# kokizzu/dragonboat

Hardware: AMD Instinct MI355X
Metric: committed entries/sec (node) at 1M active 3-replica groups, 16B payload; %HBM BW (higher is better)
Workload: dtype u64

## Files before the change

dragonboat_amd/abi.py:

```python
import ctypes as C

DRB_MAX_REPLICAS = 8
DRB_RI_DEPTH = 4
DRB_NONE = 0xFFFFFFFF

DRB_OK = 0
DRB_EINVAL = -1
DRB_EDEVICE = -2
DRB_ENOMEM = -3
DRB_ENOSYS = -4
DRB_ERANGE = -5
DRB_EAGAIN = -6
DRB_EDIVERTED = -7

MSG = dict(
    LocalTick=0, Election=1, LeaderHeartbeat=2, ConfigChangeEvent=3, NoOP=4,
    Ping=5, Pong=6, Propose=7, SnapshotStatus=8, Unreachable=9,
    CheckQuorum=10, BatchedReadIndex=11, Replicate=12, ReplicateResp=13,
    RequestVote=14, RequestVoteResp=15, InstallSnapshot=16, Heartbeat=17,
    HeartbeatResp=18, ReadIndex=19, ReadIndexResp=20, Quiesce=21,
    SnapshotReceived=22, LeaderTransfer=23, TimeoutNow=24, RateLimit=25,
    RequestPreVote=26, RequestPreVoteResp=27, LogQuery=28)
MSG_NAME = {v: k for k, v in MSG.items()}

# ... 77 lines not shown
                ("hint_high", C.c_uint64), ("type", C.c_uint32),
                ("reject", C.c_uint32), ("n_entries", C.c_uint64),
                ("entries_off", C.c_uint64)]


class ReadyToRead(C.Structure):
    _fields_ = [("shard_id", C.c_uint64), ("replica_id", C.c_uint64),
                ("index", C.c_uint64), ("ctx_low", C.c_uint64),
                ("ctx_high", C.c_uint64)]


class Config(C.Structure):
    _fields_ = [("num_groups", C.c_uint64), ("first_shard_id", C.c_uint64),
                ("num_replicas", C.c_uint32), ("window", C.c_uint32),
                ("cmd_cap", C.c_uint32), ("max_props", C.c_uint32),
                ("prop_slots", C.c_uint32), ("ri_slots", C.c_uint32),
                ("mailbox", C.c_uint32), ("kv_slots", C.c_uint32),
                ("kv_val_cap", C.c_uint32), ("election_rtt", C.c_uint32),
                ("heartbeat_rtt", C.c_uint32), ("check_quorum", C.c_uint32),
                ("device", C.c_int32), ("save_cap", C.c_uint32),
                ("total_groups", C.c_uint64), ("place_world", C.c_uint32),
                ("place_rank", C.c_uint32), ("entry_mbox", C.c_uint32),
                ("kv_pool_blocks", C.c_uint32), ("flagged_cap", C.c_uint32),
                ("quiesce", C.c_uint32), ("durable_log", C.c_uint32),
                ("save_batched", C.c_uint32), ("save_tan", C.c_uint32),
                ("elections", C.c_uint32), ("tan_max_log", C.c_uint64),
                ("tan_multiplexed", C.c_uint32), ("pre_vote", C.c_uint32),
                ("max_reads_per_ctx", C.c_uint32),
                ("kv_overflow_buckets", C.c_uint64),
                ("forward_proposals", C.c_uint32),
                ("nonvoting_slots", C.c_uint32),
                ("witness_slots", C.c_uint32),
                ("host_copies", C.c_uint32), ("no_lean", C.c_uint32),
                ("entry_compression", C.c_uint32),
                ("session_slots", C.c_uint32),
                ("session_history", C.c_uint32)]


class ReadResult(C.Structure):
    _fields_ = [("shard_id", C.c_uint64), ("index", C.c_uint64),
                ("ctx_low", C.c_uint64), ("ctx_high", C.c_uint64),
                ("key", C.c_uint64), ("replica_id", C.c_uint32),
                ("read", C.c_uint32), ("found", C.c_uint32),
                ("vlen", C.c_uint32), ("value", C.c_uint32),
                ("pad", C.c_uint32)]


class ApplyResult(C.Structure):
    _fields_ = [("group", C.c_uint64), ("index", C.c_uint64),
                ("key", C.c_uint64), ("client_id", C.c_uint64),
                ("series_id", C.c_uint64), ("value", C.c_uint64),
                ("slot", C.c_uint32), ("ignored", C.c_uint32)]


APPLY_IGNORED, APPLY_REJECTED = 1, 2

SERIES_REGISTER, SERIES_UNREGISTER = 2 ** 64 - 2, 2 ** 64 - 1


class SessionRec(C.Structure):
    _fields_ = [("client_id", C.c_uint64), ("responded_up_to", C.c_uint64),
                ("n_history", C.c_uint32), ("first_history", C.c_uint32)]


class SessionResp(C.Structure):
    _fields_ = [("series_id", C.c_uint64), ("value", C.c_uint64)]
# ... 224 lines not shown
```

dragonboat_amd/csrc/drb_engine.hip:

```cpp
#include <hip/hip_runtime.h>
#include <stdio.h>
#include <stdlib.h>
#include <string.h>

#include <algorithm>
#include <memory>
#include <mutex>
#include <unordered_map>
#include <vector>

#include <hipcub/hipcub.hpp>

#include "../../include/drb_engine.h"
#include "drb_layout.hpp"
#include "drb_msg.hpp"
#include "drb_place.hpp"
#include "drb_rows.hpp"
#include "drb_step.hpp"
#include "drb_launch.hpp"
#include "drb_hsa.hpp"
#include "drb_res.hpp"

using namespace drb;

#define HIPCHK(x)                                                        \
  do {                                                                   \
    hipError_t e_ = (x);                                                 \
    if (e_ != hipSuccess) {                                              \
      fprintf(stderr, "drb_engine: %s failed: %s (%s:%d)\n", #x,          \
              hipGetErrorString(e_), __FILE__, __LINE__);                \
      return DRB_EDEVICE;                                                \
    }                                                                    \
  } while (0)

struct drb_engine {
  drb_config cfg;
  View v;
  View *dview;
  Stream stream;
  Stream stream2;
  Event ev_fork, ev_join;
  Stream stream_h2d;
  HsaXfer xfer;
  int failed = 0;
  DevBuf sess_client;
  bool no_lean = false;
  std::vector<drb_engine *> bound;
  std::vector<PeerPlanes> peers_host;
  Event ev_staged;
  Event ev_stage_free;
  Event ev_uploaded;
  Event ev_xsend, ev_xrecv;
  uint64_t exchanged_round = 0;
  std::vector<Event> ev_prop;
  uint64_t round = 0;
  uint64_t ticks = 0;
  uint64_t committed_round = 0;
  uint64_t bytes = 0;
  std::vector<DevBuf> allocs;
  uint64_t ctr_rows = 0;
  uint32_t *xcount = nullptr;
  uint32_t role_slots[2] = {0, 0};
  uint32_t *role_dev = nullptr;
  unsigned long long *ctr_total = nullptr;
  DevBuf scratch;
  DevBuf stage_buf;
  struct WireState *wire = nullptr;
  struct IngestState *ingest = nullptr;
  struct WorkerState *worker = nullptr;
  std::mutex ingest_mu;
  bool crc_tab_ready = false;
  uint64_t tan_blocks = 0;
  uint64_t tan_wblocks = 0;
  uint32_t *tan_list = nullptr;
  uint32_t *tan_n = nullptr;
  uint32_t tan_per_list = 0;
  unsigned long long *tan_total = nullptr;
  uint64_t reads_round = ~0ull;
  uint32_t reads_n = 0, reads_ks = 0;
  DevBuf xout;
  unsigned long long *xpull_bytes = nullptr;
  uint64_t xcopy_bytes = 0;
  bool xrows_used = false;
  std::vector<bool> recovered;
};

static void wire_free(drb_engine *e);
// ... 104 lines not shown
  if (cfg->cmd_cap == 0 || cfg->cmd_cap % 16 || cfg->cmd_cap > 1040)
    return DRB_ENOSYS;
  if (cfg->mailbox < 4 || cfg->mailbox > MB_MAX) return DRB_EINVAL;
  if (!is_pow2(cfg->kv_slots) || cfg->kv_val_cap == 0 ||
      cfg->kv_val_cap > 1024)
    return DRB_EINVAL;
  if (cfg->max_props == 0 || cfg->prop_slots == 0 || cfg->ri_slots == 0)
    return DRB_EINVAL;
  if (cfg->save_cap % 16) return DRB_EINVAL;
  if (cfg->save_batched && (cfg->save_cap == 0 || cfg->window < 64))
    return DRB_EINVAL;
  if (cfg->save_tan && (cfg->save_cap == 0 || cfg->save_batched))
    return DRB_EINVAL;
  if (cfg->pre_vote && !cfg->elections) return DRB_EINVAL;
  if (cfg->tan_multiplexed && (!cfg->save_tan || cfg->place_world > 1))
    return DRB_EINVAL;
  if (cfg->save_tan && (uint64_t)cfg->num_replicas * cfg->num_groups > 0xffffffffull)
    return DRB_ERANGE;
  if (cfg->place_world > 1 &&
      (cfg->place_rank >= cfg->place_world || cfg->entry_mbox == 0 ||
       cfg->entry_mbox > cfg->window || cfg->entry_mbox > 255))
    return DRB_EINVAL;
  if (cfg->election_rtt == 0 || cfg->heartbeat_rtt == 0) return DRB_EINVAL;
  if ((cfg->nonvoting_slots & cfg->witness_slots) ||
      ((cfg->nonvoting_slots | cfg->witness_slots) >> cfg->num_replicas) ||
      __builtin_popcount(cfg->nonvoting_slots | cfg->witness_slots) >=
          (int)cfg->num_replicas)
    return DRB_EINVAL;
  if (cfg->forward_proposals &&
      (cfg->max_props > MAX_FWD_PROPS || cfg->place_world > 1))
    return DRB_EINVAL;
  if ((uint64_t)cfg->window * (128 + cfg->cmd_cap) > MAX_ENTRY_SIZE)
    return DRB_EINVAL;
  if (cfg->host_copies > 1 || cfg->entry_compression > 1) return DRB_EINVAL;
  if (cfg->session_slots > SESS_MAX_SLOTS ||
      (cfg->session_slots ? cfg->session_history == 0 ||
                                cfg->session_history > SESS_MAX_HISTORY
                          : cfg->session_history != 0))
    return DRB_EINVAL;
  if (cfg->total_groups >
      cfg->num_groups * std::max<uint64_t>(cfg->place_world, 1))
    return DRB_EINVAL;
  if (cfg->kv_overflow_buckets >= 0xffffffffull) return DRB_ERANGE;
  if (cfg->save_tan && cfg->tan_multiplexed &&
      (uint64_t)tanm_records(cfg->num_groups) * cfg->save_cap > 0xffffffffull)
    return DRB_ERANGE;
  return DRB_OK;
}

namespace {
struct EngineDestroy {
  void operator()(drb_engine *e) const { (void)drb_engine_destroy(e); }
};
}

extern "C" int drb_engine_create(const drb_config *cfg, drb_engine **out) {
  if (!cfg || !out) return DRB_EINVAL;
  *out = nullptr;
  if (int rc = validate_config(cfg)) return rc;
  std::unique_ptr<drb_engine, EngineDestroy> owner(new drb_engine());
  drb_engine *e = owner.get();
  e->cfg = *cfg;
  if (cfg->host_copies) e->xfer.state = -1;
  e->no_lean = cfg->no_lean != 0;
  if (hipSetDevice(cfg->device) != hipSuccess ||
      e->stream.create() != hipSuccess || e->stream2.create() != hipSuccess ||
      e->stream_h2d.create() != hipSuccess)
    return DRB_EDEVICE;
  e->ev_prop.resize(cfg->prop_slots);
  for (Event *ev : {&e->ev_fork, &e->ev_join, &e->ev_staged, &e->ev_stage_free,
                    &e->ev_uploaded, &e->ev_xsend, &e->ev_xrecv})
    if (ev->create() != hipSuccess) return DRB_EDEVICE;
  for (Event &ev : e->ev_prop)
    if (ev.create() != hipSuccess) return DRB_EDEVICE;
  View &v = e->v;
  memset(&v, 0, sizeof(v));
  const uint64_t G = cfg->num_groups, R = cfg->num_replicas;
  v.G = G;
  v.R = (uint32_t)R;
  v.W = cfg->window;
  v.C16 = cfg->cmd_cap / 16;
  v.MB = cfg->mailbox;
  v.KS = cfg->kv_slots;
  v.kv_val_cap = cfg->kv_val_cap;
  v.kv_ool = cfg->kv_val_cap > 124;
  v.KVW = v.kv_ool ? 2
                   : 1 + (cfg->kv_val_cap > 4 ? (cfg->kv_val_cap - 4 + 15) / 16
                                              : 0);
  v.VB = v.kv_ool ? (cfg->kv_val_cap + 15) / 16 : 0;
  v.kv_pool_blocks =
      v.kv_ool ? (cfg->kv_pool_blocks
                      ? cfg->kv_pool_blocks
                      : std::min<uint64_t>(G * R * v.KS +
                                               4 * cfg->kv_overflow_buckets,
                                           0xffffffffull))
               : 0;
  v.max_props = cfg->max_props;
  v.election_rtt = cfg->election_rtt;
  v.heartbeat_rtt = cfg->heartbeat_rtt;
// ... 674 lines not shown
  if (!e || slot >= e->v.R) return DRB_EINVAL;
  k_host_slot<<<(unsigned)((e->v.G + 255) / 256), 256, 0, e->stream>>>(
      e->v, slot, hosted ? 1u : 0u);
  HIPCHK(hipGetLastError());
  return refresh_roles(e);
}

DRB_DEV void stage_row(const View &v, uint32_t slot, uint32_t j, uint64_t g,
                       const drb_entry &en, const uint8_t *cmd,
                       bool readable) {
  uint4 meta[PROP_META];
  const bool held = prop_pack(v, en, cmd, readable, meta);
  for (uint32_t c = 0; c < PROP_META; ++c)
    v.props[prop_ix(v, slot, j, c, g)] = meta[c];
  for (uint32_t c = 0; held && c < v.C16; ++c)
    v.props[prop_ix(v, slot, j, PROP_META + c, g)] =
        cmd_chunk(cmd, en.cmd_len, c);
}

__global__ void k_stage_props(View v, uint32_t slot, const uint32_t *counts,
                              const drb_entry *ents, const uint8_t *pool,
                              uint64_t pool_len) {
  const uint64_t g = (uint64_t)blockIdx.x * blockDim.x + threadIdx.x;
  if (g >= v.G) return;
  const uint32_t n = counts[g];
  v.prop_count[(uint64_t)slot * v.G + g] = n;
  for (uint32_t j = 0; j < n; ++j) {
    const drb_entry en = ents[g * v.max_props + j];
    stage_row(v, slot, j, g, en, pool + en.cmd_off,
              en.cmd_off + en.cmd_len <= pool_len);
  }
}

extern "C" int drb_stage_proposals(drb_engine *e, uint32_t slot,
                                   const uint32_t *counts,
                                   const drb_entry *ents,
                                   const uint8_t *pool, size_t pool_len) {
  if (!e || slot >= e->cfg.prop_slots) return DRB_ERANGE;
  if (!counts || !ents || (pool_len && !pool)) return DRB_EINVAL;
  const View &v = e->v;
  const uint64_t G = v.G;
  for (uint64_t g = 0; g < G; ++g)
    if (counts[g] > v.max_props) return DRB_ERANGE;
  const size_t ent_b = (size_t)G * v.max_props * sizeof(drb_entry);
  const size_t cnt_off = ent_b, pool_off = (cnt_off + G * 4 + 255) & ~(size_t)255;
  const size_t need = pool_off + std::max<uint64_t>(pool_len, 16);
  if (need > e->stage_buf.cap) {
    HIPCHK(hipStreamSynchronize(e->stream));
    HIPCHK(hipStreamSynchronize(e->stream_h2d));
    if (e->stage_buf.reserve(need)) return DRB_EDEVICE;
  }
  uint8_t *d = e->stage_buf.as<uint8_t>();
  HIPCHK(hipStreamWaitEvent(e->stream_h2d, e->ev_stage_free, 0));
  HIPCHK(hipMemcpyAsync(d, ents, ent_b, hipMemcpyHostToDevice,
                        e->stream_h2d));
  HIPCHK(hipMemcpyAsync(d + cnt_off, counts, G * 4, hipMemcpyHostToDevice,
                        e->stream_h2d));
  if (pool_len)
    HIPCHK(hipMemcpyAsync(d + pool_off, pool, pool_len, hipMemcpyHostToDevice,
                          e->stream_h2d));
  HIPCHK(hipEventRecord(e->ev_staged, e->stream_h2d));
  HIPCHK(hipStreamWaitEvent(e->stream, e->ev_staged, 0));
  k_stage_props<<<(unsigned)((G + 255) / 256), 256, 0, e->stream>>>(
      v, slot, (const uint32_t *)(d + cnt_off), (const drb_entry *)d,
      d + pool_off, (uint64_t)pool_len);
  HIPCHK(hipGetLastError());
  HIPCHK(hipEventRecord(e->ev_stage_free, e->stream));
  HIPCHK(hipEventRecord(e->ev_prop[slot], e->stream));
  HIPCHK(hipEventSynchronize(e->ev_staged));
  return DRB_OK;
}

// ... 29 lines not shown
  }
}

constexpr size_t kSdmaMinBytes = 8u << 20;

static void stage_layout(uint64_t G, uint64_t n, size_t pool_len,
                         uint64_t off[4], size_t *bytes) {
  auto al = [](size_t x) { return (x + 255) & ~(size_t)255; };
  const uint64_t n1 = n ? n : 1;
  off[0] = al(G);
  off[2] = off[0] + al(8 * n1);
  off[3] = off[2] + al(2 * n1);
  off[1] = al(off[3] + pool_len);
  *bytes = off[1] + 8 * n1;
}

extern "C" int drb_stage_packed_layout(const drb_engine *e, uint64_t n_entries,
                                       size_t pool_len, uint64_t *offsets,
                                       size_t *bytes) {
  if (!e || !offsets || !bytes) return DRB_EINVAL;
  stage_layout(e->v.G, n_entries, pool_len, offsets, bytes);
  return DRB_OK;
}

static int stage_packed(drb_engine *e, uint32_t slot, uint32_t type,
                        const uint8_t *counts, uint64_t n_entries,
                        const uint64_t *keys, const uint64_t *client_ids,
                        const uint16_t *cmd_lens, const uint8_t *pool,
                        size_t pool_len, bool async) {
  if (!e || slot >= e->cfg.prop_slots) return DRB_ERANGE;
  if (!counts || (n_entries && (!keys || !cmd_lens)) || (pool_len && !pool))
    return DRB_EINVAL;
  if (n_entries && !client_ids && !e->sess_client.p) return DRB_EINVAL;
  const View &v = e->v;
  const uint64_t G = v.G, n = n_entries;
  uint64_t tsum = 0;
  uint32_t cmax = 0;
  for (uint64_t g = 0; g < G; ++g) {
    cmax = std::max<uint32_t>(cmax, counts[g]);
    tsum += counts[g];
  }
  if (cmax > v.max_props) return DRB_ERANGE;
  if (tsum != n) return DRB_EINVAL;
  auto al = [](size_t x) { return (x + 255) & ~(size_t)255; };
  const uint64_t n1 = n ? n : 1;
  size_t tb1 = 0, tb2 = 0;
  HIPCHK(hipcub::DeviceScan::ExclusiveSum(
      nullptr, tb1, WidenU8((const uint8_t *)nullptr, WidenU32()),
      (uint32_t *)nullptr, (int)G, e->stream));
  HIPCHK(hipcub::DeviceScan::ExclusiveSum(
      nullptr, tb2, WidenU16((const uint16_t *)nullptr, WidenU32()),
      (uint32_t *)nullptr, (int)n1, e->stream));
  uint64_t lo[4];
  size_t up = 0;
  stage_layout(G, n, pool_len, lo, &up);
  const size_t o_cnt = 0, o_key = lo[0], o_cid = lo[1], o_len = lo[2],
               o_pool = lo[3];
  if (!client_ids) up = o_pool + pool_len;
  const size_t o_e0 = al(std::max<size_t>(up, o_pool + 16)),
               o_off = o_e0 + al(4 * G), o_tmp = o_off + al(4 * n1),
               need = o_tmp + al(std::max(tb1, tb2));
  if (need > e->stage_buf.cap) {
    HIPCHK(hipStreamSynchronize(e->stream));
    HIPCHK(hipStreamSynchronize(e->stream_h2d));
    if (e->stage_buf.reserve(need)) return DRB_EDEVICE;
  }
// ... 182 lines not shown
      const bool on =
          mix64(seed ^ ACTIVE_SALT ^ (g * 0x9E3779B97F4A7C15ull) ^
                (salt << 24)) % 1000000u < active_ppm;
      v.prop_count[(uint64_t)ps * v.G + lane] = on ? k : 0u;
      if (on) list[atomicAdd(&nlist, 1u)] = (uint32_t)(lane - base);
    }
    __syncthreads();
    const uint32_t n = nlist;
    if (n >= 256 || it + 1 == GEN_ITERS) {
      if (threadIdx.x < n && threadIdx.x < 256)
        gen_kv_lane(v, ps, k, key_space, val_len, seed, salt,
                    base + list[threadIdx.x]);
      __syncthreads();
      if (n > 256 && threadIdx.x < n - 256)
        list[threadIdx.x] = list[256 + threadIdx.x];
      if (threadIdx.x == 0) nlist = n > 256 ? n - 256 : 0u;
      __syncthreads();
    }
  }
  const uint32_t n = nlist;
  if (threadIdx.x < n)
    gen_kv_lane(v, ps, k, key_space, val_len, seed, salt,
                base + list[threadIdx.x]);
}

extern "C" int drb_gen_kv_proposals_active(drb_engine *e, uint32_t slot,
                                           uint32_t k, uint32_t key_space,
                                           uint32_t val_len, uint64_t seed,
                                           uint64_t salt, uint32_t active_ppm) {
  if (!e || slot >= e->cfg.prop_slots || k > e->cfg.max_props || !key_space ||
      val_len > 16383 ||
      12 + (val_len < 128 ? 1 : 2) + val_len > e->cfg.cmd_cap)
    return DRB_EINVAL;
  const uint64_t per = active_ppm >= 1000000u ? 256 : GEN_ITERS * 256;
  k_gen_kv<<<(unsigned)((e->v.G + per - 1) / per), 256, 0, e->stream>>>(
      e->v, slot, k, key_space, val_len, seed, salt, active_ppm);
  HIPCHK(hipGetLastError());
  HIPCHK(hipEventRecord(e->ev_prop[slot], e->stream));
  return DRB_OK;
}

extern "C" int drb_gen_kv_proposals(drb_engine *e, uint32_t slot, uint32_t k,
                                    uint32_t key_space, uint32_t val_len,
                                    uint64_t seed, uint64_t salt) {
  return drb_gen_kv_proposals_active(e, slot, k, key_space, val_len, seed,
                                     salt, 1000000u);
}

extern "C" int drb_stage_read_index(drb_engine *e, uint32_t slot,
                                    const uint64_t *ctx_low,
                                    const uint64_t *ctx_high) {
  if (!e || slot >= e->cfg.ri_slots) return DRB_ERANGE;
  const uint64_t G = e->v.G;
  std::vector<uint4> host(G);
  for (uint64_t g = 0; g < G; ++g) host[g] = pack2(ctx_low[g], ctx_high[g]);
  HIPCHK(hipMemcpyAsync(e->v.ri_in + (uint64_t)slot * G, host.data(),
                        G * sizeof(uint4), hipMemcpyHostToDevice, e->stream));
  HIPCHK(hipStreamSynchronize(e->stream));
  return DRB_OK;
}

__global__ void k_gen_ri(View v, uint32_t rs, uint64_t seed, uint64_t salt,
                         uint64_t high) {
  const uint64_t lane = (uint64_t)blockIdx.x * blockDim.x + threadIdx.x;
  if (lane >= v.G) return;
  const uint64_t g = gid(v, v.stage_slot, lane);
  uint64_t low = mix64(seed ^ 0x5EAD1DE85EAD1DE8ull ^
                       (g * 0x9E3779B97F4A7C15ull) ^ (salt << 40)) |
                 1;
  v.ri_in[(uint64_t)rs * v.G + lane] = mk4(low, high);
}
// ... 463 lines not shown
      for (int k = 0; k < NUM_STEP_KINDS; ++k)
        fn[R - 1][k] = fn[R - 1][step_kind_at(R, k)];
  }
};
static constexpr StepLaunchTable kStepLaunch;

static int launch_step(drb_engine *e, const RoundParams &p0,
                       hipStream_t st = nullptr, uint32_t blk0 = 0,
                       uint32_t nblk = 0) {
  const unsigned gx_all = (unsigned)((e->v.G + 255) / 256);
  const unsigned gx = nblk ? nblk : gx_all;
  if (!st) st = e->stream;
  if (e->v.R < 1 || e->v.R > 8) return DRB_EINVAL;
  if (p0.listed) {
    switch (e->v.R) {
#define DRB_X(R, K) \
  case R: k_active_scan<R><<<gx, 256, 0, e->stream>>>(e->v, p0); break;
      DRB_FOR_ALL_R(DRB_X, )
#undef DRB_X
    }
    k_active_prefix<<<4 * e->v.R, 1024, 0, e->stream>>>(e->v, gx);
    k_active_scatter<<<dim3(gx, e->v.R), 256, 0, e->stream>>>(e->v);
  }
  RoundParams pl = p0, pf = p0;
  pl.blk0 = pf.blk0 = blk0;
  pl.gx_all = pf.gx_all = nblk ? gx_all : 0u;
  uint32_t nl = 0, nf = 0;
  pl.slots = slot_list(e->role_slots[0], &nl);
  pf.slots = slot_list(e->role_slots[1], &nf);
  pl.nrows = nl;
  pf.nrows = nf;
  const StepPlan plan =
      plan_step(e->v, p0.encode_saves, p0.listed, nl, nf, gx,
                !nblk && st == e->stream, e->no_lean);
  const StepLaunchFn *launch = kStepLaunch.fn[e->v.R - 1];
  if (plan.split) {
    (void)hipEventRecord(e->ev_fork, st);
    (void)hipStreamWaitEvent(e->stream2, e->ev_fork, 0);
  }
  if (plan.lean) {
    if (plan.split) {
      (void)hipEventRecord(e->ev_join, e->stream2);
      (void)hipStreamWaitEvent(st, e->ev_join, 0);
    }
    if (nl) launch[SK_LEAD_LEAN](e->v, pl, gx * nl, st);
    if (nf) launch[SK_FOLLOW_LEAN](e->v, pf, gx * nf, st);
    pl.lean = pf.lean = LEAN_ALL;
    if (nl) launch[plan.lead](e->v, pl, gx * nl, st);
    if (nf) launch[plan.follow](e->v, pf, gx * nf, st);
  } else {
    if (nl) launch[plan.lead](e->v, pl, gx * nl, st);
    if (nf)
      launch[plan.follow](e->v, pf, gx * nf, plan.split ? e->stream2 : st);
    if (plan.split) {
      (void)hipEventRecord(e->ev_join, e->stream2);
      (void)hipStreamWaitEvent(st, e->ev_join, 0);
    }
    if (plan.slow) {
      RoundParams ps = p0;
      ps.slots = 0;
      ps.nrows = 1;
      launch[SK_SLOW](e->v, ps, (e->v.slow_cap + 255) / 256, e->stream);
    }
  }
  HIPCHK(hipGetLastError());
  return DRB_OK;
}
// ... 33 lines not shown
  __syncthreads();
  const uint64_t g = (uint64_t)blockIdx.x * blockDim.x + threadIdx.x;
  const uint32_t s = blockIdx.y;
  if (g < v.G) {
    const uint32_t fl = v.u32[u32_ix(v, W_FLAGS, s, g)];
    if ((fl & DRB_F_HOSTED) && !(fl & (DRB_F_FALLBACK | DRB_F_ERROR)))
      atomicAdd(&part[v.u32[u32_ix(v, W_ROLE, s, g)] & 7u], 1ull);
  }
  __syncthreads();
  if (threadIdx.x < 8 && part[threadIdx.x])
    atomicAdd(&out[s * 8 + threadIdx.x], part[threadIdx.x]);
}

extern "C" int drb_role_census(drb_engine *e, uint64_t *counts) {
  if (!e || !counts) return DRB_EINVAL;
  void *d;
  const size_t bytes = (size_t)e->v.R * 8 * sizeof(uint64_t);
  if (scratch(e, bytes, &d)) return DRB_EDEVICE;
  HIPCHK(hipMemsetAsync(d, 0, bytes, e->stream));
  dim3 grid((unsigned)((e->v.G + 255) / 256), e->v.R);
  k_role_census<<<grid, 256, 0, e->stream>>>(e->v,
                                             (unsigned long long *)d);
  HIPCHK(hipGetLastError());
  HIPCHK(hipMemcpyAsync(counts, d, bytes, hipMemcpyDeviceToHost, e->stream));
  HIPCHK(hipStreamSynchronize(e->stream));
  return DRB_OK;
}

extern "C" int drb_role_slots(const drb_engine *e, uint32_t *leader_slots,
                              uint32_t *follower_slots) {
  if (!e) return DRB_EINVAL;
  if (leader_slots) *leader_slots = e->role_slots[0];
  if (follower_slots) *follower_slots = e->role_slots[1];
  return DRB_OK;
}

static int round_params(drb_engine *e, const drb_round_in *in, uint64_t ahead,
                        uint64_t ticks_before, RoundParams *out) {
  if (in->prop_slot != DRB_NONE && in->prop_slot >= e->cfg.prop_slots)
    return DRB_ERANGE;
  if (in->ri_slot != DRB_NONE && in->ri_slot >= e->cfg.ri_slots)
    return DRB_ERANGE;
  RoundParams p;
  memset(&p, 0, sizeof(p));
  p.slots = 0;
  p.nrows = 1;
  p.round = e->round + 1 + ahead;
  p.tick = in->tick ? 1 : 0;
  p.tick_no = ticks_before + p.tick;
  p.prop_slot = in->prop_slot;
  p.ri_slot = in->ri_slot;
  p.n_reads = in->reads_per_ctx;
  p.key_space = in->read_key_space;
  if (p.n_reads && !p.key_space) return DRB_EINVAL;
  if (p.n_reads && e->v.max_reads && p.n_reads > e->v.max_reads)
    return DRB_ERANGE;
  p.encode_saves = in->encode_saves ? 1 : 0;
  if (p.encode_saves && !e->v.save_cap16) return DRB_EINVAL;
  p.ri_replica = in->ri_replica;
  p.listed = in->listed ? 1 : 0;
  if (p.listed && e->v.remote_mask) return DRB_EINVAL;
  p.prop_replica = in->prop_replica;
  if (p.prop_replica > e->v.R || (p.prop_replica && !e->v.fwd_props))
    return DRB_EINVAL;
  if (p.ri_replica > e->v.R || (p.ri_replica && e->v.place_world > 1))
    return DRB_EINVAL;
// ... 6 lines not shown

static void round_done(drb_engine *e, const RoundParams &p) {
  e->round++;
  e->ticks += p.tick;
  if (p.n_reads) {
    e->reads_round = e->round;
    e->reads_n = p.n_reads;
    e->reads_ks = p.key_space;
  }
}

extern "C" int drb_step_round_async(drb_engine *e, const drb_round_in *in) {
  if (!e || !in) return DRB_EINVAL;
  std::lock_guard<std::mutex> ingest_lock(e->ingest_mu);
  if (e->failed) return e->failed;
  if (e->cfg.durable_log && e->committed_round < e->round) return DRB_EINVAL;
  RoundParams p;
  if (int rc = round_params(e, in, 0, e->ticks, &p)) return rc;
  if (e->v.elections)
    HIPCHK(hipMemsetAsync(e->v.slow_n, 0, 8, e->stream));
  if (e->v.remote_mask && e->xrows_used)
    HIPCHK(hipMemsetAsync(e->v.xrows, 0,
                          2ull * e->v.R * e->v.R * ((e->v.G + 255) / 256) * 4,
                          e->stream));
  if (e->v.xslow && e->xrows_used)
    HIPCHK(hipMemsetAsync(e->v.xslow, 0,
                          4ull * e->v.R * e->v.R * ((e->v.G + 255) / 256) * 4,
                          e->stream));
  if (int rc = launch_step(e, p)) return rc;
  if (p.encode_saves && e->v.save_tan) {
    int rc = launch_tan(e, (uint32_t)p.round);
    if (rc) return rc;
  }
  if (p.prop_slot != DRB_NONE)
    HIPCHK(hipEventRecord(e->ev_prop[p.prop_slot], e->stream));
  round_done(e, p);
  return DRB_OK;
}

extern "C" int drb_step_rounds(drb_engine *e, const drb_round_in *in,
                               uint32_t k, uint64_t chunk_groups) {
  if (!e || !in || !k) return DRB_EINVAL;
  std::lock_guard<std::mutex> ingest_lock(e->ingest_mu);
  if (e->failed) return e->failed;
  if (e->v.elections || e->v.remote_mask || e->v.save_tan ||
      e->cfg.durable_log)
    return DRB_EINVAL;
  const uint64_t gx = (e->v.G + 255) / 256;
  if (!chunk_groups || chunk_groups % 256) return DRB_EINVAL;
  const uint64_t cb = chunk_groups / 256;
  std::vector<RoundParams> ps(k);
  uint64_t ticks = e->ticks;
  for (uint32_t t = 0; t < k; ++t) {
    if (in[t].listed) return DRB_EINVAL;
    if (int rc = round_params(e, &in[t], t, ticks, &ps[t])) return rc;
    ticks += ps[t].tick;
  }
  HIPCHK(hipEventRecord(e->ev_fork, e->stream));
  HIPCHK(hipStreamWaitEvent(e->stream2, e->ev_fork, 0));
  int rc = DRB_OK;
  if (cb >= gx) {
    for (uint32_t t = 0; t < k && !rc; ++t) rc = launch_step(e, ps[t]);
  } else {
    for (uint64_t c0 = 0, c = 0; c0 < gx && !rc; c0 += cb, ++c) {
      const uint32_t nb = (uint32_t)std::min<uint64_t>(cb, gx - c0);
      hipStream_t st = (c & 1) ? e->stream2 : e->stream;
      for (uint32_t t = 0; t < k && !rc; ++t)
        rc = launch_step(e, ps[t], st, (uint32_t)c0, nb);
    }
  }
  const hipError_t j1 = hipEventRecord(e->ev_join, e->stream2);
  const hipError_t j2 = hipStreamWaitEvent(e->stream, e->ev_join, 0);
  if (rc || j1 != hipSuccess || j2 != hipSuccess) {
    e->failed = rc ? rc : DRB_EDEVICE;
    return e->failed;
  }
  for (uint32_t t = 0; t < k; ++t) {
    if (ps[t].prop_slot != DRB_NONE)
      HIPCHK(hipEventRecord(e->ev_prop[ps[t].prop_slot], e->stream));
    round_done(e, ps[t]);
  }
  return DRB_OK;
}

__global__ void k_sum_counters(const unsigned long long *rows, uint64_t n,
                               unsigned long long *total) {
  __shared__ unsigned long long part[256];
  for (int c = 0; c < NUM_COUNTERS; ++c) {
    unsigned long long s = 0;
    for (uint64_t r = threadIdx.x; r < n; r += blockDim.x)
      s += rows[r * NUM_COUNTERS + c];
    part[threadIdx.x] = s;
    __syncthreads();
    for (int o = 128; o > 0; o >>= 1) {
      if (threadIdx.x < (unsigned)o) part[threadIdx.x] += part[threadIdx.x + o];
      __syncthreads();
    }
    if (threadIdx.x == 0) total[c] = part[0];
    __syncthreads();
  }
}

extern "C" int drb_debug_phase(drb_engine *e, uint64_t *out, int reset) {
  if (!e || !out) return DRB_EINVAL;
  memset(out, 0, 16 * sizeof(uint64_t));
  if (!e->v.phase) return DRB_OK;
  HIPCHK(hipMemcpyAsync(out, e->v.phase, 16 * sizeof(uint64_t),
                        hipMemcpyDeviceToHost, e->stream));
  if (reset)
    HIPCHK(hipMemsetAsync(e->v.phase, 0, 16 * sizeof(uint64_t), e->stream));
  HIPCHK(hipStreamSynchronize(e->stream));
  return DRB_OK;
// ... 2229 lines not shown
```

dragonboat_amd/csrc/drb_kinds.hpp:

```cpp
#pragma once
#include "drb_layout.hpp"

namespace drb {

#define DRB_FOR_ALL_R(X, K) \
  X(1, K) X(2, K) X(3, K) X(4, K) X(5, K) X(6, K) X(7, K) X(8, K)
#define DRB_FOR_R3_R5(X, K) X(3, K) X(5, K)

#define DRB_STEP_KINDS(X)                                                  \
  X(LEAD, 0, STEP, 1, 0, 0, 0, 0, ALL_R, LEAD)                             \
  X(LEAD_EXT, 1, STEP, 1, 1, 0, 0, 0, ALL_R, LEAD_EXT)                     \
  X(FOLLOW, 2, STEP, 0, 0, 0, 0, 0, ALL_R, FOLLOW)                         \
  X(FOLLOW_EXT, 3, STEP, 0, 1, 0, 0, 0, ALL_R, FOLLOW_EXT)                 \
  X(SLOW, 4, STEP, 1, 1, 1, 1, 0, ALL_R, SLOW)                             \
  X(LEAD_FWD, 5, STEP, 1, 1, 0, 1, 0, ALL_R, LEAD_FWD)                     \
  X(FOLLOW_FWD, 6, STEP, 0, 1, 0, 1, 0, ALL_R, FOLLOW_FWD)                 \
  X(LEAD_LEAN, 7, LEAN, 1, 0, 0, 0, 0, ALL_R, LEAD_LEAN)                   \
  X(FOLLOW_LEAN, 8, LEAN, 0, 0, 0, 0, 0, ALL_R, FOLLOW_LEAN)               \
  X(LEAD_LOCAL, 9, STEP, 1, 0, 0, 0, 1, R3_R5, LEAD)                       \
  X(FOLLOW_LOCAL, 10, STEP, 0, 0, 0, 0, 1, R3_R5, FOLLOW)                  \
  X(LEAD_EXT_LOCAL, 11, STEP, 1, 1, 0, 0, 1, R3_R5, LEAD_EXT)              \
  X(FOLLOW_EXT_LOCAL, 12, STEP, 0, 1, 0, 0, 1, R3_R5, FOLLOW_EXT)

enum StepKind : int {
#define DRB_X(name, num, ...) SK_##name = num,
  DRB_STEP_KINDS(DRB_X)
#undef DRB_X
  NUM_STEP_KINDS
};

enum StepKernel { SKN_STEP, SKN_LEAN };

struct StepKindInfo {
  StepKernel kernel;
  bool lead, ext, slow, fwd, local;
  uint32_t built_for;
  int stand_in;
};

constexpr StepKindInfo kStepKinds[NUM_STEP_KINDS] = {
#define DRB_X_BIT(R, K) | 1u << R
#define DRB_X(name, num, kernel, L, E, S, F, LOC, set, alt)              \
  {SKN_##kernel, L != 0, E != 0, S != 0, F != 0, LOC != 0,               \
   0u DRB_FOR_##set(DRB_X_BIT, num), SK_##alt},
    DRB_STEP_KINDS(DRB_X)
#undef DRB_X
#undef DRB_X_BIT
};

constexpr int step_kind_at(int R, int kind) {
  return (kStepKinds[kind].built_for >> R) & 1u ? kind
                                                : kStepKinds[kind].stand_in;
}

constexpr uint64_t kSplitMaxBlocks = 2048;

struct StepPlan {
  int lead, follow;
  bool split;
  bool lean;
  bool slow;
};

inline StepPlan plan_step(const View &v, bool encode_saves, bool listed,
                          uint32_t nl, uint32_t nf, unsigned gx,
                          bool whole_round_on_engine_stream, bool no_lean) {
  const bool ext = v.C16 > 4 || v.kv_ool || encode_saves || v.quiesce ||
                   v.kv_ovf_cap || v.snappy || v.sessions;
  const bool fwd = v.fwd_props || v.nv_mask || v.wt_mask;
  const bool local = !v.remote_mask;
  StepPlan p;
  p.lead = fwd ? SK_LEAD_FWD
           : ext ? (local ? SK_LEAD_EXT_LOCAL : SK_LEAD_EXT)
                 : (local ? SK_LEAD_LOCAL : SK_LEAD);
  p.follow = fwd ? SK_FOLLOW_FWD
             : ext ? (local ? SK_FOLLOW_EXT_LOCAL : SK_FOLLOW_EXT)
                   : (local ? SK_FOLLOW_LOCAL : SK_FOLLOW);
  p.split = nl && nf && whole_round_on_engine_stream && !v.elections &&
            (uint64_t)gx * (nl + nf) <= kSplitMaxBlocks;
  p.lean = listed && ext && !fwd && whole_round_on_engine_stream &&
           !v.elections && local && !v.save_tan && !v.save_batched &&
           !no_lean;
  p.slow = v.elections != 0;
  return p;
}

}
```

dragonboat_amd/csrc/drb_res.hpp:

```cpp
#pragma once

#include <stddef.h>

#include <utility>

namespace drb {

template <class A>
struct Buf {
  void *p = nullptr;
  size_t cap = 0;

  Buf() = default;
  Buf(Buf &&o) noexcept : p(o.p), cap(o.cap) { o.p = nullptr, o.cap = 0; }
  Buf &operator=(Buf &&o) noexcept {
    if (this != &o) {
      reset();
      std::swap(p, o.p);
      std::swap(cap, o.cap);
    }
    return *this;
  }
  ~Buf() { reset(); }

// ... 54 lines not shown
static inline int hip_alloc_rc(hipError_t r, const char *what, size_t bytes) {
  if (r != hipSuccess)
    fprintf(stderr, "drb_engine: %s of %zu bytes failed: %s\n", what, bytes,
            hipGetErrorString(r));
  return r != hipSuccess;
}
struct HipDevice {
  static int alloc(void **p, size_t n) {
    return hip_alloc_rc(hipMalloc(p, n), "hipMalloc", n);
  }
  static void free(void *p) { (void)hipFree(p); }
};
template <unsigned Flags>
struct HipPinned {
  static int alloc(void **p, size_t n) {
    return hip_alloc_rc(hipHostMalloc(p, n, Flags), "hipHostMalloc", n);
  }
  static void free(void *p) { (void)hipHostFree(p); }
};
using DevBuf = Buf<HipDevice>;
template <unsigned Flags>
using PinnedBuf = Buf<HipPinned<Flags>>;

struct StreamDestroy {
  static bool null(hipStream_t s) { return !s; }
  static void destroy(hipStream_t s) { (void)hipStreamDestroy(s); }
};
struct Stream : Handle<hipStream_t, StreamDestroy> {
  hipError_t create() {
    const hipError_t r = hipStreamCreateWithFlags(out(), hipStreamNonBlocking);
    if (r != hipSuccess) h = nullptr;
    return r;
  }
};
struct EventDestroy {
  static bool null(hipEvent_t e) { return !e; }
  static void destroy(hipEvent_t e) { (void)hipEventDestroy(e); }
};
struct Event : Handle<hipEvent_t, EventDestroy> {
  hipError_t create(unsigned flags = hipEventDisableTiming) {
    const hipError_t r = hipEventCreateWithFlags(out(), flags);
    if (r != hipSuccess) h = nullptr;
    return r;
  }
};
struct SignalDestroy {
  static bool null(hsa_signal_t s) { return !s.handle; }
  static void destroy(hsa_signal_t s) { (void)hsa_signal_destroy(s); }
};
struct Signal : Handle<hsa_signal_t, SignalDestroy> {
  hsa_status_t create() {
    const hsa_status_t r = hsa_signal_create(0, 0, nullptr, out());
    if (r != HSA_STATUS_SUCCESS) h = hsa_signal_t{0};
    return r;
  }
};

}
#endif
```

dragonboat_amd/engine.py:

```python
import ctypes as C
import os

from . import abi
from .abi import (ApplyResult, Config, Entry, Flagged, Message, ReadyToRead, Region, ReplicaState,
                  RoundIn, RoundOut, WireCfg, WireCpu, WireIn, WireOut,
                  entry_to_tuple,
                  message_to_tuple)

HERE = os.path.dirname(os.path.abspath(__file__))
LIB_PATH = os.environ.get("DRB_ENGINE_LIB") or \
    os.path.join(HERE, "_lib", "libdrb_engine.so")

_lib = None

P = C.c_void_p
U64 = C.c_uint64
U32 = C.c_uint32
PU64 = C.POINTER(C.c_uint64)
PU32 = C.POINTER(C.c_uint32)
PU8 = C.POINTER(C.c_uint8)
SZ = C.c_size_t

SIGNATURES = {
    "drb_engine_create": (C.c_int, [C.POINTER(Config), C.POINTER(P)]),
    "drb_engine_destroy": (C.c_int, [P]),
    "drb_engine_device_bytes": (U64, [P]),
    "drb_engine_stream": (P, [P]),
    "drb_engine_sync": (C.c_int, [P]),
    "drb_engine_round": (U64, [P]),
    "drb_import_replicas": (C.c_int, [P, U64, U64,
                                      C.POINTER(ReplicaState)]),
    "drb_export_replicas": (C.c_int, [P, U64, U64,
                                      C.POINTER(ReplicaState)]),
    "drb_import_log": (C.c_int, [P, U64, U32, C.POINTER(Entry), SZ, PU8]),
    "drb_export_log": (C.c_int, [P, U64, U32, U64, U64, C.POINTER(Entry),
                                 PU8, SZ]),
    "drb_init_steady": (C.c_int, [P, U64, U32, U64]),
    "drb_host_slot": (C.c_int, [P, U32, C.c_int]),
    "drb_role_census": (C.c_int, [P, PU64]),
    "drb_export_save_records": (C.c_int, [P, U64, U32,
                                          C.POINTER(abi.SaveRecord), SZ,
                                          C.POINTER(SZ)]),
    "drb_role_slots": (C.c_int, [P, PU32, PU32]),
    "drb_stage_proposals": (C.c_int, [P, U32, PU32, C.POINTER(Entry), PU8,
                                      SZ]),
    "drb_stage_proposals_packed": (C.c_int, [P, U32, U32, PU8, U64, PU64,
                                             PU64, C.POINTER(C.c_uint16),
                                             PU8, SZ]),
    "drb_stage_proposals_packed_async": (C.c_int, [P, U32, U32, PU8, U64, PU64,
                                             PU64, C.POINTER(C.c_uint16),
                                             PU8, SZ]),
    "drb_stage_wait_upload": (C.c_int, [P]),
    "drb_set_session_clients": (C.c_int, [P, PU64]),
    "drb_stage_packed_layout": (C.c_int, [P, U64, SZ, PU64, C.POINTER(SZ)]),
    "drb_gen_kv_proposals": (C.c_int, [P, U32, U32, U32, U32, U64, U64]),
    "drb_gen_kv_proposals_active": (C.c_int, [P, U32, U32, U32, U32, U64,
                                              U64, U32]),
    "drb_stage_read_index": (C.c_int, [P, U32, PU64, PU64]),
    "drb_gen_read_index": (C.c_int, [P, U32, U64, U64]),
    "drb_request_leader_transfer": (C.c_int, [P, U32, PU32, PU64]),
    "drb_ingest": (C.c_int, [P, C.POINTER(Message), SZ, C.POINTER(Entry),
                             PU8, PU64, PU64]),
    "drb_ingest_ex": (C.c_int, [P, C.POINTER(Message), SZ, C.POINTER(Entry),
                                PU8, PU8, PU64, PU64, PU64]),
    "drb_export_inbox": (C.c_int, [P, U64, U32, C.c_int, C.POINTER(Message),
                                   SZ, C.POINTER(Entry), SZ, PU8, SZ,
                                   C.POINTER(SZ)]),
    "drb_ingest_wire_cpu": (C.c_int, [P, C.POINTER(WireCpu), SZ,
                                      C.POINTER(SZ)]),
    "drb_step_round": (C.c_int, [P, C.POINTER(RoundIn),
                                 C.POINTER(RoundOut)]),
    "drb_step_round_async": (C.c_int, [P, C.POINTER(RoundIn)]),
    "drb_step_rounds": (C.c_int, [P, C.POINTER(RoundIn), U32, U64]),
    "drb_read_counters": (C.c_int, [P, C.POINTER(RoundOut), C.c_int]),
    "drb_debug_phase": (C.c_int, [P, C.POINTER(U64), C.c_int]),
    "drb_take_flagged": (C.c_int, [P, C.POINTER(Flagged), SZ, C.POINTER(SZ),
# ... 121 lines not shown
    n = SZ(0)
    _ck(lib().drb_payload_decode(type, _u8(cmd), len(cmd), out, cap,
                                 C.byref(n)), "drb_payload_decode")
    return bytes(out[:n.value])


def tan_scan(data, cap=None):
    data = bytes(data)
    n, oc, vend = SZ(0), C.c_int(0), U64(0)
    buf = _u8(data)
    want = 64 if cap is None else cap
    while True:
        out = (abi.TanScanRec * max(1, want))()
        _ck(lib().drb_tan_scan(buf, len(data), out, want, C.byref(n),
                               C.byref(oc), C.byref(vend)), "drb_tan_scan")
        if cap is not None or n.value <= want:
            break
        want = n.value
    recs = [{f: getattr(out[i], f) for f, _ in abi.TanScanRec._fields_}
            for i in range(min(n.value, want))]
    return oc.value, vend.value, recs


DEFAULTS = dict(num_groups=1, first_shard_id=1, num_replicas=3, window=32,
                cmd_cap=32, max_props=4, prop_slots=2, ri_slots=2,
                mailbox=16, kv_slots=512, kv_val_cap=4, election_rtt=10,
                heartbeat_rtt=1, check_quorum=1, device=0, save_cap=0,
                total_groups=0, place_world=1, place_rank=0, entry_mbox=0,
                kv_pool_blocks=0, flagged_cap=0, quiesce=0, durable_log=0,
                save_batched=0, save_tan=0, tan_max_log=0, elections=0,
                tan_multiplexed=0, pre_vote=0, max_reads_per_ctx=0,
                kv_overflow_buckets=0, forward_proposals=0,
                nonvoting_slots=0, witness_slots=0, host_copies=0,
                no_lean=0, entry_compression=0, session_slots=0,
                session_history=0)


class Engine:

    def __init__(self, **kw):
        cfg = dict(DEFAULTS)
        cfg.update(kw)
        self.cfg = cfg
        c = Config(cfg["num_groups"], cfg["first_shard_id"],
                   cfg["num_replicas"], cfg["window"], cfg["cmd_cap"],
                   cfg["max_props"], cfg["prop_slots"], cfg["ri_slots"],
                   cfg["mailbox"], cfg["kv_slots"], cfg["kv_val_cap"],
                   cfg["election_rtt"], cfg["heartbeat_rtt"],
                   cfg["check_quorum"], cfg["device"], cfg["save_cap"],
                   cfg["total_groups"], cfg["place_world"], cfg["place_rank"],
                   cfg["entry_mbox"], cfg["kv_pool_blocks"],
                   cfg["flagged_cap"], cfg["quiesce"],
                   cfg["durable_log"], cfg["save_batched"],
                   cfg["save_tan"], cfg["elections"], cfg["tan_max_log"],
                   cfg["tan_multiplexed"], cfg["pre_vote"],
                   cfg["max_reads_per_ctx"], cfg["kv_overflow_buckets"],
                   cfg["forward_proposals"], cfg["nonvoting_slots"],
                   cfg["witness_slots"], cfg["host_copies"],
                   cfg["no_lean"], cfg["entry_compression"],
                   cfg["session_slots"], cfg["session_history"])
        h = P()
        _ck(lib().drb_engine_create(C.byref(c), C.byref(h)),
            "drb_engine_create")
        self.h = h
        self.G = cfg["num_groups"]
        self.R = cfg["num_replicas"]

    def close(self):
        if getattr(self, "h", None):
            lib().drb_engine_destroy(self.h)
            self.h = None

    def __del__(self):
        self.close()

    @property
    def device_bytes(self):
        return lib().drb_engine_device_bytes(self.h)

    @property
    def round(self):
        return lib().drb_engine_round(self.h)

    @property
    def stream(self):
        return lib().drb_engine_stream(self.h)

    def sync(self):
        _ck(lib().drb_engine_sync(self.h), "drb_engine_sync")

    def import_replicas(self, first_group, states):
        n = len(states) // self.R
        arr = (ReplicaState * len(states))(*states)
        _ck(lib().drb_import_replicas(self.h, first_group, n, arr),
            "drb_import_replicas")

    def export_replicas(self, first_group, n_groups):
        arr = (ReplicaState * (n_groups * self.R))()
        _ck(lib().drb_export_replicas(self.h, first_group, n_groups, arr),
            "drb_export_replicas")
        return list(arr)

    def export(self, g, slot):
        return self.export_replicas(g, 1)[slot]

    def import_log(self, g, slot, entries, pool):
        _ck(lib().drb_import_log(self.h, g, slot, entries, len(entries), pool),
            "drb_import_log")

    def export_log(self, g, slot, lo, hi):
        n = hi - lo + 1
        if n <= 0:
            return []
        arr = (Entry * n)()
        pcap = n * self.cfg["cmd_cap"] + 16
        pool = (C.c_uint8 * pcap)()
        _ck(lib().drb_export_log(self.h, g, slot, lo, hi, arr, pool, pcap),
            "drb_export_log")
        return [entry_to_tuple(arr[i], pool) for i in range(n)]

    def role_slots(self):
        a, b = U32(), U32()
        _ck(lib().drb_role_slots(self.h, C.byref(a), C.byref(b)),
            "drb_role_slots")
        return a.value, b.value

    def host_slot(self, slot, hosted):
        _ck(lib().drb_host_slot(self.h, slot, int(bool(hosted))),
            "drb_host_slot")

    def init_steady(self, term=2, leader_slot=0, seed=0x5EEDD8B0):
        _ck(lib().drb_init_steady(self.h, term, leader_slot, seed),
            "drb_init_steady")

    def stage_proposals(self, slot, counts, ents, pool, pool_len=None):
        if pool_len is None:
            pool_len = C.sizeof(pool)
        _ck(lib().drb_stage_proposals(self.h, slot, counts, ents, pool,
                                      pool_len), "drb_stage_proposals")

    def stage_proposals_packed(self, slot, type, counts, n, keys, clients,
                               lens, pool, pool_len):
        _ck(lib().drb_stage_proposals_packed(self.h, slot, type, counts, n,
                                             keys, clients, lens, pool,
                                             pool_len),
            "drb_stage_proposals_packed")

    def stage_proposals_packed_async(self, slot, type, counts, n, keys,
                                     clients, lens, pool, pool_len):
        _ck(lib().drb_stage_proposals_packed_async(
            self.h, slot, type, counts, n, keys, clients, lens, pool,
            pool_len), "drb_stage_proposals_packed_async")

    def stage_packed_layout(self, n_entries, pool_len):
        off = (U64 * 4)()
        nb = SZ()
        _ck(lib().drb_stage_packed_layout(self.h, n_entries, pool_len, off,
                                          C.byref(nb)),
# ... 576 lines not shown
```

include/drb_engine.h:

```cpp
#ifndef DRB_ENGINE_H
#define DRB_ENGINE_H

#include <stddef.h>
#include <stdint.h>

#ifdef __cplusplus
extern "C" {
#endif

#define DRB_MAX_REPLICAS 8
#define DRB_RI_DEPTH 4

#define DRB_OK 0
#define DRB_EINVAL (-1)
#define DRB_EDEVICE (-2)
#define DRB_ENOMEM (-3)
#define DRB_ENOSYS (-4)
#define DRB_ERANGE (-5)
#define DRB_EAGAIN (-6)
#define DRB_EDIVERTED (-7)

enum drb_message_type {
  DRB_MSG_LOCAL_TICK = 0,
  DRB_MSG_ELECTION = 1,
// ... 176 lines not shown
  uint32_t cmd_cap;
  uint32_t max_props;
  uint32_t prop_slots;
  uint32_t ri_slots;
  uint32_t mailbox;
  uint32_t kv_slots;
  uint32_t kv_val_cap;
  uint32_t election_rtt;
  uint32_t heartbeat_rtt;
  uint32_t check_quorum;
  int32_t device;
  uint32_t save_cap;
  uint64_t total_groups;
  uint32_t place_world;
  uint32_t place_rank;
  uint32_t entry_mbox;
  uint32_t kv_pool_blocks;
  uint32_t flagged_cap;
  uint32_t quiesce;
  uint32_t durable_log;
  uint32_t save_batched;
  uint32_t save_tan;
  uint32_t elections;
  uint64_t tan_max_log;
  uint32_t tan_multiplexed;
  uint32_t pre_vote;
  uint32_t max_reads_per_ctx;
  uint64_t kv_overflow_buckets;
  uint32_t forward_proposals;
  uint32_t nonvoting_slots;
  uint32_t witness_slots;
  uint32_t host_copies;
  uint32_t no_lean;
  uint32_t entry_compression;
  uint32_t session_slots;
  uint32_t session_history;
} drb_config;

typedef struct drb_round_in {
  uint32_t tick;
  uint32_t prop_slot;
  uint32_t ri_slot;
  uint32_t reads_per_ctx;
  uint32_t read_key_space;
  uint32_t encode_saves;
  uint32_t ri_replica;
  uint32_t listed;
  uint32_t prop_replica;
} drb_round_in;

#define DRB_NONE 0xffffffffu

typedef struct drb_round_out {
  uint64_t round;
  uint64_t committed_entries;
  uint64_t applied_entries;
  uint64_t messages;
  uint64_t ready_to_reads;
  uint64_t dropped_read_indexes;
  uint64_t fallbacks;
  uint64_t errors;
  uint64_t reads_served;
  uint64_t reads_deferred;
  uint64_t saved_entries;
  uint64_t saved_bytes;
  uint64_t replicas_stepped;
// ... 214 lines not shown
  uint64_t end_offset;
  uint64_t bytes;
  uint32_t start_log;
  uint32_t end_log;
  uint32_t flags;
  uint32_t pad;
} drb_tan_log;
int drb_export_tan_log(drb_engine *e, uint32_t slot, uint32_t key,
                       drb_tan_log *out, uint8_t *buf, size_t cap);
int drb_tan_buffers(drb_engine *e, void **bytes, void **recs);

int drb_saved_buffers(drb_engine *e, void **bytes, uint32_t **lens,
                      uint32_t **crcs);

typedef struct drb_region {
  void *ptr;
  uint64_t bytes;
} drb_region;

#define DRB_PLANE_REGIONS 10
#define DRB_PLANE_KREP(w) ((w) & 0x1fu)
#define DRB_PLANE_KOTH(w) (((w) >> 5) & 0x1fu)
#define DRB_PLANE_E(w) (((w) >> 10) & 0xffu)
#define DRB_PLANE_C1 (1u << 18)
#define DRB_PLANE_HDR (1u << 19)
#define DRB_PLANE_TOTHER (1u << 20)

int drb_plane_counts(drb_engine *e, uint32_t *words);
int drb_plane_peer(const drb_engine *e, uint32_t from, uint32_t to, int dir);
int drb_place_peer(uint32_t world, uint32_t rank, uint32_t from, uint32_t to,
                   int dir);
int drb_role_slots(const drb_engine *e, uint32_t *leader_slots,
                   uint32_t *follower_slots);
int drb_plane_regions(drb_engine *e, uint32_t from, uint32_t to,
                      uint32_t word, int dir, drb_region *out);
int drb_exchange_local(drb_engine *const *engines, uint32_t n);
int drb_exchange_local_bind(drb_engine *const *engines, uint32_t n);
typedef struct drb_xfer {
  uint32_t peer;
  uint32_t recv;
  void *ptr;
  uint64_t bytes;
} drb_xfer;
int drb_exchange_plan(drb_engine *e, uint32_t leader_mask, drb_xfer *xfers,
                      size_t cap, size_t *n_xfers);
int drb_exchange_rccl(drb_engine *e, void *comm, uint32_t leader_mask);
int drb_exchange_plan_words(drb_engine *e, const uint32_t *words,
                            drb_xfer *xfers, size_t cap, size_t *n_xfers);
int drb_exchange_rccl_counted(drb_engine *e, void *comm);
int drb_exchange_rccl_roles(drb_engine *e, void *comm, uint32_t *leader_mask);
int drb_exchange_bytes(drb_engine *e, uint64_t *bytes, int reset);
int drb_exchange_local_counted(drb_engine *const *engines, uint32_t n);
int drb_exchange_mark(drb_engine *e);

#define DRB_APPLY_IGNORED 1u
#define DRB_APPLY_REJECTED 2u
typedef struct drb_apply_result {
  uint64_t group;
  uint64_t index;
  uint64_t key;
  uint64_t client_id;
  uint64_t series_id;
  uint64_t value;
  uint32_t slot;
  uint32_t ignored;
} drb_apply_result;
// ... 173 lines not shown
```

Measured before the change: 1.020 billion.

## Add round_overlap option with priority streams and tail-split step form

Adds a round_overlap config (and DRB_ROUND_OVERLAP env override) that selects how leader and follower step kernels are split across two streams, including a new tail-split form. The streams are now created with high and low priority when the device supports it. Proposal-slot event records are skipped until host staging is first used, which removes one event record per round on the device-generated proposal path. The default keeps the tail form disabled, so the default behaviour mostly changes through stream priorities and the skipped event records.

```diff
diff --git a/dragonboat_amd/abi.py b/dragonboat_amd/abi.py
--- a/dragonboat_amd/abi.py
+++ b/dragonboat_amd/abi.py
@@ -133,6 +133,7 @@
                 ("nonvoting_slots", C.c_uint32),
                 ("witness_slots", C.c_uint32),
                 ("host_copies", C.c_uint32), ("no_lean", C.c_uint32),
+                ("round_overlap", C.c_uint32),
                 ("entry_compression", C.c_uint32),
                 ("session_slots", C.c_uint32),
                 ("session_history", C.c_uint32)]
diff --git a/dragonboat_amd/csrc/drb_engine.hip b/dragonboat_amd/csrc/drb_engine.hip
--- a/dragonboat_amd/csrc/drb_engine.hip
+++ b/dragonboat_amd/csrc/drb_engine.hip
@@ -39,6 +39,7 @@
   View *dview;
   Stream stream;
   Stream stream2;
+  bool prio_streams = false;
   Event ev_fork, ev_join;
   Stream stream_h2d;
   HsaXfer xfer;
@@ -53,6 +54,7 @@
   Event ev_xsend, ev_xrecv;
   uint64_t exchanged_round = 0;
   std::vector<Event> ev_prop;
+  bool host_staging = false;
   uint64_t round = 0;
   uint64_t ticks = 0;
   uint64_t committed_round = 0;
@@ -223,7 +225,9 @@
     return DRB_EINVAL;
   if ((uint64_t)cfg->window * (128 + cfg->cmd_cap) > MAX_ENTRY_SIZE)
     return DRB_EINVAL;
-  if (cfg->host_copies > 1 || cfg->entry_compression > 1) return DRB_EINVAL;
+  if (cfg->host_copies > 1 || cfg->entry_compression > 1 ||
+      cfg->round_overlap > 2)
+    return DRB_EINVAL;
   if (cfg->session_slots > SESS_MAX_SLOTS ||
       (cfg->session_slots ? cfg->session_history == 0 ||
                                 cfg->session_history > SESS_MAX_HISTORY
@@ -254,8 +258,19 @@
   e->cfg = *cfg;
   if (cfg->host_copies) e->xfer.state = -1;
   e->no_lean = cfg->no_lean != 0;
-  if (hipSetDevice(cfg->device) != hipSuccess ||
-      e->stream.create() != hipSuccess || e->stream2.create() != hipSuccess ||
+  if (const char *ro = getenv("DRB_ROUND_OVERLAP"))
+    if (!cfg->round_overlap && (ro[0] == '1' || ro[0] == '2') && !ro[1])
+      e->cfg.round_overlap = (uint32_t)(ro[0] - '0');
+  if (hipSetDevice(cfg->device) != hipSuccess) return DRB_EDEVICE;
+  int prio_least = 0, prio_greatest = 0;
+  if (hipDeviceGetStreamPriorityRange(&prio_least, &prio_greatest) !=
+      hipSuccess)
+    prio_least = prio_greatest = 0;
+  e->prio_streams = prio_greatest < prio_least;
+  if ((e->prio_streams ? e->stream.create(prio_greatest)
+                       : e->stream.create()) != hipSuccess ||
+      (e->prio_streams ? e->stream2.create(prio_least)
+                       : e->stream2.create()) != hipSuccess ||
       e->stream_h2d.create() != hipSuccess)
     return DRB_EDEVICE;
   e->ev_prop.resize(cfg->prop_slots);
@@ -996,12 +1011,26 @@
   }
 }
 
+static hipError_t mark_prop(drb_engine *e, uint32_t slot) {
+  return e->host_staging ? hipEventRecord(e->ev_prop[slot], e->stream)
+                         : hipSuccess;
+}
+
+static int host_staging_begin(drb_engine *e) {
+  std::lock_guard<std::mutex> lock(e->ingest_mu);
+  if (e->host_staging) return DRB_OK;
+  for (Event &ev : e->ev_prop) HIPCHK(hipEventRecord(ev, e->stream));
+  e->host_staging = true;
+  return DRB_OK;
+}
+
 extern "C" int drb_stage_proposals(drb_engine *e, uint32_t slot,
                                    const uint32_t *counts,
                                    const drb_entry *ents,
                                    const uint8_t *pool, size_t pool_len) {
   if (!e || slot >= e->cfg.prop_slots) return DRB_ERANGE;
   if (!counts || !ents || (pool_len && !pool)) return DRB_EINVAL;
+  if (int rc = host_staging_begin(e)) return rc;
   const View &v = e->v;
   const uint64_t G = v.G;
   for (uint64_t g = 0; g < G; ++g)
@@ -1097,6 +1126,7 @@
   if (!counts || (n_entries && (!keys || !cmd_lens)) || (pool_len && !pool))
     return DRB_EINVAL;
   if (n_entries && !client_ids && !e->sess_client.p) return DRB_EINVAL;
+  if (int rc = host_staging_begin(e)) return rc;
   const View &v = e->v;
   const uint64_t G = v.G, n = n_entries;
   uint64_t tsum = 0;
@@ -1345,11 +1375,12 @@
       val_len > 16383 ||
       12 + (val_len < 128 ? 1 : 2) + val_len > e->cfg.cmd_cap)
     return DRB_EINVAL;
+  std::lock_guard<std::mutex> lock(e->ingest_mu);
   const uint64_t per = active_ppm >= 1000000u ? 256 : GEN_ITERS * 256;
   k_gen_kv<<<(unsigned)((e->v.G + per - 1) / per), 256, 0, e->stream>>>(
       e->v, slot, k, key_space, val_len, seed, salt, active_ppm);
   HIPCHK(hipGetLastError());
-  HIPCHK(hipEventRecord(e->ev_prop[slot], e->stream));
+  HIPCHK(mark_prop(e, slot));
   return DRB_OK;
 }
 
@@ -1879,7 +1910,8 @@
   pf.nrows = nf;
   const StepPlan plan =
       plan_step(e->v, p0.encode_saves, p0.listed, nl, nf, gx,
-                !nblk && st == e->stream, e->no_lean);
+                !nblk && st == e->stream, e->no_lean, e->cfg.round_overlap,
+                e->prio_streams);
   const StepLaunchFn *launch = kStepLaunch.fn[e->v.R - 1];
   if (plan.split) {
     (void)hipEventRecord(e->ev_fork, st);
@@ -1979,6 +2011,19 @@
   if (!e) return DRB_EINVAL;
   if (leader_slots) *leader_slots = e->role_slots[0];
   if (follower_slots) *follower_slots = e->role_slots[1];
+  return DRB_OK;
+}
+
+extern "C" int drb_round_form(const drb_engine *e, uint32_t listed,
+                              uint32_t *form) {
+  if (!e || !form) return DRB_EINVAL;
+  uint32_t nl = 0, nf = 0;
+  (void)slot_list(e->role_slots[0], &nl);
+  (void)slot_list(e->role_slots[1], &nf);
+  *form = plan_step(e->v, false, listed != 0, nl, nf,
+                    (unsigned)((e->v.G + 255) / 256), true, e->no_lean,
+                    e->cfg.round_overlap, e->prio_streams)
+              .split;
   return DRB_OK;
 }
 
@@ -2051,8 +2096,7 @@
     int rc = launch_tan(e, (uint32_t)p.round);
     if (rc) return rc;
   }
-  if (p.prop_slot != DRB_NONE)
-    HIPCHK(hipEventRecord(e->ev_prop[p.prop_slot], e->stream));
+  if (p.prop_slot != DRB_NONE) HIPCHK(mark_prop(e, p.prop_slot));
   round_done(e, p);
   return DRB_OK;
 }
@@ -2095,8 +2139,7 @@
     return e->failed;
   }
   for (uint32_t t = 0; t < k; ++t) {
-    if (ps[t].prop_slot != DRB_NONE)
-      HIPCHK(hipEventRecord(e->ev_prop[ps[t].prop_slot], e->stream));
+    if (ps[t].prop_slot != DRB_NONE) HIPCHK(mark_prop(e, ps[t].prop_slot));
     round_done(e, ps[t]);
   }
   return DRB_OK;
diff --git a/dragonboat_amd/csrc/drb_kinds.hpp b/dragonboat_amd/csrc/drb_kinds.hpp
--- a/dragonboat_amd/csrc/drb_kinds.hpp
+++ b/dragonboat_amd/csrc/drb_kinds.hpp
@@ -55,16 +55,26 @@
 
 constexpr uint64_t kSplitMaxBlocks = 2048;
 
+enum SplitForm : int {
+  SPLIT_NONE = 0,
+  SPLIT_SIDE = 1,
+  SPLIT_TAIL = 2,
+};
+
+constexpr bool kTailFillDefault = false;
+
 struct StepPlan {
   int lead, follow;
-  bool split;
+  SplitForm split;
   bool lean;
   bool slow;
 };
 
 inline StepPlan plan_step(const View &v, bool encode_saves, bool listed,
                           uint32_t nl, uint32_t nf, unsigned gx,
-                          bool whole_round_on_engine_stream, bool no_lean) {
+                          bool whole_round_on_engine_stream, bool no_lean,
+                          uint32_t round_overlap = 0,
+                          bool prio_streams = false) {
   const bool ext = v.C16 > 4 || v.kv_ool || encode_saves || v.quiesce ||
                    v.kv_ovf_cap || v.snappy || v.sessions;
   const bool fwd = v.fwd_props || v.nv_mask || v.wt_mask;
@@ -76,8 +86,16 @@
   p.follow = fwd ? SK_FOLLOW_FWD
              : ext ? (local ? SK_FOLLOW_EXT_LOCAL : SK_FOLLOW_EXT)
                    : (local ? SK_FOLLOW_LOCAL : SK_FOLLOW);
-  p.split = nl && nf && whole_round_on_engine_stream && !v.elections &&
-            (uint64_t)gx * (nl + nf) <= kSplitMaxBlocks;
+  const bool both = nl && nf && whole_round_on_engine_stream && !v.elections;
+  const bool small = (uint64_t)gx * (nl + nf) <= kSplitMaxBlocks;
+  const bool tail_round = both && !listed && local;
+  p.split = round_overlap == 1               ? SPLIT_NONE
+            : round_overlap == 2 && tail_round ? SPLIT_TAIL
+            : both && small                  ? SPLIT_SIDE
+            : kTailFillDefault && round_overlap == 0 && prio_streams &&
+                    tail_round
+                ? SPLIT_TAIL
+                : SPLIT_NONE;
   p.lean = listed && ext && !fwd && whole_round_on_engine_stream &&
            !v.elections && local && !v.save_tan && !v.save_batched &&
            !no_lean;
diff --git a/dragonboat_amd/csrc/drb_res.hpp b/dragonboat_amd/csrc/drb_res.hpp
--- a/dragonboat_amd/csrc/drb_res.hpp
+++ b/dragonboat_amd/csrc/drb_res.hpp
@@ -110,6 +110,12 @@
     if (r != hipSuccess) h = nullptr;
     return r;
   }
+  hipError_t create(int priority) {
+    const hipError_t r =
+        hipStreamCreateWithPriority(out(), hipStreamNonBlocking, priority);
+    if (r != hipSuccess) h = nullptr;
+    return r;
+  }
 };
 struct EventDestroy {
   static bool null(hipEvent_t e) { return !e; }
diff --git a/dragonboat_amd/engine.py b/dragonboat_amd/engine.py
--- a/dragonboat_amd/engine.py
+++ b/dragonboat_amd/engine.py
@@ -42,6 +42,7 @@
                                           C.POINTER(abi.SaveRecord), SZ,
                                           C.POINTER(SZ)]),
     "drb_role_slots": (C.c_int, [P, PU32, PU32]),
+    "drb_round_form": (C.c_int, [P, U32, PU32]),
     "drb_stage_proposals": (C.c_int, [P, U32, PU32, C.POINTER(Entry), PU8,
                                       SZ]),
     "drb_stage_proposals_packed": (C.c_int, [P, U32, U32, PU8, U64, PU64,
@@ -229,8 +230,8 @@
                 tan_multiplexed=0, pre_vote=0, max_reads_per_ctx=0,
                 kv_overflow_buckets=0, forward_proposals=0,
                 nonvoting_slots=0, witness_slots=0, host_copies=0,
-                no_lean=0, entry_compression=0, session_slots=0,
-                session_history=0)
+                no_lean=0, round_overlap=0, entry_compression=0,
+                session_slots=0, session_history=0)
 
 
 class Engine:
@@ -254,7 +255,8 @@
                    cfg["max_reads_per_ctx"], cfg["kv_overflow_buckets"],
                    cfg["forward_proposals"], cfg["nonvoting_slots"],
                    cfg["witness_slots"], cfg["host_copies"],
-                   cfg["no_lean"], cfg["entry_compression"],
+                   cfg["no_lean"], cfg["round_overlap"],
+                   cfg["entry_compression"],
                    cfg["session_slots"], cfg["session_history"])
         h = P()
         _ck(lib().drb_engine_create(C.byref(c), C.byref(h)),
@@ -321,6 +323,12 @@
         _ck(lib().drb_role_slots(self.h, C.byref(a), C.byref(b)),
             "drb_role_slots")
         return a.value, b.value
+
+    def round_form(self, listed=False):
+        f = U32()
+        _ck(lib().drb_round_form(self.h, int(bool(listed)), C.byref(f)),
+            "drb_round_form")
+        return f.value
 
     def host_slot(self, slot, hosted):
         _ck(lib().drb_host_slot(self.h, slot, int(bool(hosted))),
diff --git a/include/drb_engine.h b/include/drb_engine.h
--- a/include/drb_engine.h
+++ b/include/drb_engine.h
@@ -232,6 +232,7 @@
   uint32_t witness_slots;
   uint32_t host_copies;
   uint32_t no_lean;
+  uint32_t round_overlap;
   uint32_t entry_compression;
   uint32_t session_slots;
   uint32_t session_history;
@@ -512,6 +513,7 @@
                    int dir);
 int drb_role_slots(const drb_engine *e, uint32_t *leader_slots,
                    uint32_t *follower_slots);
+int drb_round_form(const drb_engine *e, uint32_t listed, uint32_t *form);
 int drb_plane_regions(drb_engine *e, uint32_t from, uint32_t to,
                       uint32_t word, int dir, drb_region *out);
 int drb_exchange_local(drb_engine *const *engines, uint32_t n);
```

After: 1.024 billion (median of 6 runs). Within noise of the previous version (+0.4%).
